# ubuntuslave/vo_single_camera_sos

Hardware: AMD Instinct MI355X
Metric: frame-pairs/sec (detect+match+triangulate+RANSAC) on 640x480 omni, 2000 kpts (higher is better)
Workload: dtype u8/f32/f64

## Files before the change

vo_single_camera_sos_amd/csrc/detect.hip:

```cpp
#include "common.h"

#include <type_traits>

namespace {

constexpr int kThreads = 256;
constexpr int kCandCap = 4096;
constexpr int kCandCapSmall = 2048;
constexpr int kCandCapLarge = 16384;
constexpr int kMaxMasks = 32;

__device__ __forceinline__ float sqrt_rn_normal(float x) {
  const float s = __builtin_amdgcn_sqrtf(x);
  const float s_dn = __int_as_float(__float_as_int(s) - 1), s_up = __int_as_float(__float_as_int(s) + 1);
  const float r_dn = __builtin_fmaf(-s_dn, s, x), r_up = __builtin_fmaf(-s_up, s, x);
  float r = (r_dn <= 0.0f) ? s_dn : s;
  r = (r_up > 0.0f) ? s_up : r;
  return r;
}

constexpr int kEigHalo = 3;
constexpr int kEigStripW = 64 - 2 * kEigHalo;

__device__ __forceinline__ void eig_flush(uint32_t* __restrict__ mstat_img, uint32_t bits, uint32_t omax) {
// ... 71 lines not shown
    if (t > t_last) return;
    const int y_pre = t - 2;
    const bool y_out = y_pre >= ys && y_pre < ye && y_pre >= e_lo && out_lane;
    const uint32_t o_pre = (uint32_t)(max(y_pre, 0) * cols) + (uint32_t)xc;
    const uint32_t mb_pre = y_out ? mb[o_pre] : 0u;
    {
      const int c = c_cur[P];
      const int l = left(c), r = right(c);
      hd[i2] = r - l;
      hs[i2] = (l + 2 * c) + r;
    }
    const int v = t - 1;
    if (v < e_lo - 1) return;
    {
      const int dxi = (hd[i0] + 2 * hd[i1]) + hd[i2], dyi = hs[i2] - hs[i0];
      const float dx = (float)dxi * scale, dy = (float)dyi * scale;
      const float xx = dx * dx, yy = dy * dy;
      float xy = dx * dy;
      if (v < 0 || v >= rows) xy = -xy;
      pxx[i2] = (left(xx) + xx) + right(xx);
      pxy[i2] = (left(xy) + xy) + right(xy);
      pyy[i2] = (left(yy) + yy) + right(yy);
    }
    const int y = v - 1;
    if (y < e_lo) return;
    {
      const float a = ((pxx[i0] + pxx[i1]) + pxx[i2]) * 0.5f, b = (pxy[i0] + pxy[i1]) + pxy[i2];
      const float c = ((pyy[i0] + pyy[i1]) + pyy[i2]) * 0.5f;
      const float e = (a + c) - sqrt_rn_normal(((a - c) * (a - c)) + (b * b));
      if (y_out) {
        const uint32_t bits = mb_pre & mask_all;
        if (bits != cur_bits) {
          eig_flush(mstat_img, cur_bits, cur_max);
          cur_bits = bits;
          cur_max = 0u;
        }
        cur_max = max(cur_max, sosvo_float_ordered(e));
      }
      const float el = left(e), er = right(e);
      hm[i2] = fmaxf(fmaxf(el, e), er);
      ec[i2] = e;
    }
    const int f = y - 1;
    const uint32_t mb_f = mb_prev & mask_all;
    mb_prev = mb_pre;
    if (f < f_lo || f > f_hi) return;
    {
      const float ev = ec[i1];
      const bool is_cand = out_lane && xc >= 1 && xc <= cols - 2 && ev == fmaxf(fmaxf(hm[i0], hm[i1]), hm[i2]) && ev > 0.0f &&
                           mb_f != 0u;
      const unsigned long long bal = __ballot(is_cand);
      if (bal) {
        const int pos = wpos + (int)__builtin_amdgcn_mbcnt_hi((uint32_t)(bal >> 32), __builtin_amdgcn_mbcnt_lo((uint32_t)bal, 0u));
        if (is_cand && pos < wcap) region[pos] = make_uint2(__float_as_uint(ev), (uint32_t)(f * cols + xc));
        wpos += __popcll(bal);
      }
    }
  };
  auto run = [&](auto edge_tag) __attribute__((always_inline)) {
    request(t_first);
    for (int t = t_first; t <= t_last; t += 3) {
#pragma unroll
      for (int k = 0; k < 3; ++k) c_cur[k] = c_pre[k];
      request(t + 3);
      step(std::integral_constant<int, 0>{}, edge_tag, t);
      step(std::integral_constant<int, 1>{}, edge_tag, t + 1);
      step(std::integral_constant<int, 2>{}, edge_tag, t + 2);
    }
  };
  if (edge_strip) run(std::true_type{}); else run(std::false_type{});
  if (lane == 0) wcnt[wave] = (uint32_t)wpos;
  const unsigned long long act = __ballot(out_lane && cur_bits != 0u);
  if (act) {
    const int first = __ffsll((long long)act) - 1;
    const uint32_t b0 = __shfl(cur_bits, first);
    if (__ballot(out_lane && cur_bits != 0u && cur_bits != b0) == 0ULL) {
      uint32_t om = (out_lane && cur_bits != 0u) ? cur_max : 0u;
      for (int s = 32; s > 0; s >>= 1) om = max(om, (uint32_t)__shfl_down((int)om, s));
      if (lane == 0) eig_flush(mstat_img, b0, om);
    } else {
      eig_flush(mstat_img, cur_bits, cur_max);
    }
  }
}

__global__ __launch_bounds__(kThreads) void mask_bbox_kernel(const uint32_t* __restrict__ mask_bits, int images_per_maskset,
                                                             int rows, int cols, int nmask, uint32_t* __restrict__ mstat) {
  __shared__ uint32_t sb[2][kMaxMasks];
  const int tid = threadIdx.x, y = blockIdx.x, set = blockIdx.y;
  if (tid < 2 * kMaxMasks) (&sb[0][0])[tid] = 0u;
  __syncthreads();
  const uint32_t* mb = mask_bits + ((size_t)set * rows + y) * cols;
  const uint32_t mask_all = nmask < 32 ? (1u << nmask) - 1u : 0xFFFFFFFFu;
  for (int x = tid; x < cols; x += kThreads) {
    uint32_t b = mb[x] & mask_all;
    while (b) {
      const int m = __ffs(b) - 1;
      b &= b - 1;
      atomicMax(&sb[0][m], 0xFFFFFFFFu - (uint32_t)x);
      atomicMax(&sb[1][m], (uint32_t)x + 1u);
    }
  }
  __syncthreads();
  if (tid < nmask && sb[1][tid]) {
    uint32_t* st = mstat + ((size_t)set * images_per_maskset * nmask + tid) * 5;
    atomicMax(&st[1], sb[0][tid]);
    atomicMax(&st[2], 0xFFFFFFFFu - (uint32_t)y);
    atomicMax(&st[3], sb[1][tid]);
    atomicMax(&st[4], (uint32_t)y + 1u);
  }
}

template <int LOGR, int NT>
__device__ __forceinline__ void bitonic_pass(unsigned long long* keys, int N, int k, int jtop, int tid) {
  constexpr int R = 1 << LOGR;
  const int jl = jtop >> (LOGR - 1);
  for (int t = tid; t < (N >> LOGR); t += NT) {
    const int i = ((t & ~(jl - 1)) << LOGR) | (t & (jl - 1));
    const bool desc = (i & k) == 0;
    unsigned long long v[R];
#pragma unroll
    for (int m = 0; m < R; ++m) v[m] = keys[i + m * jl];
#pragma unroll
    for (int sb = LOGR - 1; sb >= 0; --sb) {
#pragma unroll
      for (int m = 0; m < R; ++m) {
        if (m & (1 << sb)) continue;
        const unsigned long long a = v[m], b = v[m | (1 << sb)];
        const bool sw = (a < b) == desc;
        v[m] = sw ? b : a;
        v[m | (1 << sb)] = sw ? a : b;
      }
    }
#pragma unroll
    for (int m = 0; m < R; ++m) keys[i + m * jl] = v[m];
  }
}

__device__ __forceinline__ uint32_t dist2_packed(uint32_t a, uint32_t b) {
  typedef short short2v __attribute__((ext_vector_type(2)));
  const short2v d = __builtin_bit_cast(short2v, a) - __builtin_bit_cast(short2v, b);
  return (uint32_t)__builtin_amdgcn_sdot2(d, d, 0, false);
}

struct gft_regions {
  const uint2* cand;
  const uint32_t* wcnt;
  const uint32_t* mb;
  int img, m, strips, nchunks, wcap, s0, c0, ns, R;
  float thr;
};

template <int NT, class F>
__device__ __forceinline__ void gft_walk_keys(const gft_regions& g, int* s_region, int tid, F&& f) {
  const int wave = __builtin_amdgcn_readfirstlane(tid >> 6), lane = tid & 63;
  for (int rb = 0; rb < g.R; rb += NT) {
    if (rb + tid < g.R) {
      const int rg = rb + tid, c = g.c0 + rg / g.ns, sidx = g.s0 + rg % g.ns;
      s_region[tid] = min((int)g.wcnt[(g.img * g.nchunks + c) * g.strips + sidx], g.wcap);
    }
    __syncthreads();
    const int rend = min(NT, g.R - rb);
    for (int rr = wave; rr < rend; rr += NT / 64) {
      const int have = s_region[rr];
      const int rg = rb + rr, c = g.c0 + rg / g.ns, sidx = g.s0 + rg % g.ns;
      const uint2* region = g.cand + (size_t)((g.img * g.nchunks + c) * g.strips + sidx) * g.wcap;
      for (int i = lane; i < have; i += 64) {
        const uint2 r = region[i];
        if (__uint_as_float(r.x) > g.thr && ((g.mb[r.y] >> g.m) & 1u))
          f(((unsigned long long)sosvo_float_ordered(__uint_as_float(r.x)) << 32) | r.y);
      }
    }
    __syncthreads();
  }
}

template <int CAND, int NT>
__device__ __forceinline__ void gft_keep_largest(const gft_regions g, unsigned long long* keys, int* s_region, int* s_count,
                                              int* s_sel, int tid) {
  constexpr int kBits = 11, kBins = 1 << kBits, kPer = kBins / 64;
  static_assert(kBins * sizeof(uint32_t) <= CAND * sizeof(unsigned long long), "the histogram lives in the key LDS");
  uint32_t* hist = reinterpret_cast<uint32_t*>(keys);
  unsigned long long prefix = 0ULL;
  int want = CAND;
  for (int shift = 64; shift > 0;) {
    const int width = min(kBits, shift);
    const unsigned long long high = shift < 64 ? ~0ULL << shift : 0ULL;
    shift -= width;
    for (int i = tid; i < kBins; i += NT) hist[i] = 0u;
    __syncthreads();
    gft_walk_keys<NT>(g, s_region, tid, [&](unsigned long long key) {
      if ((key & high) == prefix) atomicAdd(&hist[(uint32_t)(key >> shift) & ((1u << width) - 1u)], 1u);
    });
    if (tid < 64) {
      uint32_t sum = 0u;
      for (int b = 0; b < kPer; ++b) sum += hist[tid * kPer + b];
      uint32_t incl = sum;
      for (int s = 1; s < 64; s <<= 1) {
        const uint32_t o = (uint32_t)__shfl_down((int)incl, s);
        if (tid + s < 64) incl += o;
      }
      uint32_t above = incl - sum;
      if (above < (uint32_t)want && (uint32_t)want <= incl) {
        for (int b = kPer - 1; b >= 0; --b) {
          const uint32_t c = hist[tid * kPer + b];
          if (above + c >= (uint32_t)want) {
            s_sel[0] = tid * kPer + b;
            s_sel[1] = want - (int)above;
            s_sel[2] = (int)c;
            break;
          }
          above += c;
        }
      }
    }
    __syncthreads();
    prefix |= (unsigned long long)(uint32_t)s_sel[0] << shift;
    want = s_sel[1];
    const bool whole_bin = want == s_sel[2];
    __syncthreads();
    if (whole_bin) break;
  }
// ... 26 lines not shown
  __shared__ unsigned long long lds_u64[CAND];
  __shared__ int s_count, s_accepted, s_overflow;
  __shared__ int s_region[NT];
  __shared__ int s_sel[3];
  __shared__ unsigned long long s_conf[64];
  __shared__ unsigned long long s_prior;
  __shared__ int s_ovf;
  unsigned long long* keys = lds_u64;
  uint32_t* grid = reinterpret_cast<uint32_t*>(lds_u64);
  uint32_t* acc_list = grid + 2 * kSelGridCells;
  const int tid = threadIdx.x;
  const int img = p / nmask, m = p - img * nmask;
  const uint32_t* st = mstat + (size_t)p * 5;
  const uint32_t* sb = mstat + ((size_t)(img / images_per_maskset) * images_per_maskset * nmask + m) * 5;
  uint32_t* sorted = sorted_g + (size_t)p * sorted_stride;
  if (tid == 0) {
    s_count = 0;
    s_accepted = 0;
    s_overflow = 0;
    s_prior = 0ULL;
    s_ovf = 0;
  }
  __syncthreads();
  const bool any = st[0] != 0u;
  const int bx0 = any ? max(1, (int)(0xFFFFFFFFu - sb[1])) : 0, by0 = any ? max(1, (int)(0xFFFFFFFFu - sb[2])) : 0;
  const int bx1 = any ? min(cols - 2, (int)sb[3] - 1) : -1, by1 = any ? min(rows - 2, (int)sb[4] - 1) : -1;
  const int bw = bx1 - bx0 + 1, bh = by1 - by0 + 1;
  if (any && bw > 0 && bh > 0) {
    const float thr = (float)((double)sosvo_ordered_float(st[0]) * quality);
    const uint32_t* mb = mask_bits + (size_t)(img / images_per_maskset) * rows * cols;
    const int s0 = bx0 / kEigStripW, s1 = bx1 / kEigStripW;
    const int c0 = by0 / chunk_rows, c1 = by1 / chunk_rows;
    const int ns = s1 - s0 + 1, R = (c1 - c0 + 1) * ns;
    const int wave = __builtin_amdgcn_readfirstlane(tid >> 6), lane = tid & 63;
    for (int rb = 0; rb < R; rb += NT) {
      if (rb + tid < R) {
        const int rg = rb + tid, c = c0 + rg / ns, sidx = s0 + rg % ns;
        const int have = (int)wcnt[(img * nchunks + c) * strips + sidx];
        if (have > wcap) s_overflow = 1;
        s_region[tid] = min(have, wcap);
      }
      __syncthreads();
      const int rend = min(NT, R - rb);
      for (int rr = wave; rr < rend; rr += NT / 64) {
        const int have = s_region[rr];
        const int rg = rb + rr, c = c0 + rg / ns, sidx = s0 + rg % ns;
        const uint2* region = cand + (size_t)((img * nchunks + c) * strips + sidx) * wcap;
        for (int i0 = 0; i0 < have; i0 += 64) {
          const int i = i0 + lane;
          uint2 r = make_uint2(0u, 0u);
          bool keep = false;
          if (i < have) {
            r = region[i];
            keep = __uint_as_float(r.x) > thr && ((mb[r.y] >> m) & 1u);
          }
          const unsigned long long km = __ballot(keep);
          if (km) {
            const int leader = __ffsll((long long)km) - 1;
            int slot0 = 0;
            if (lane == leader) slot0 = atomicAdd(&s_count, __popcll(km));
            slot0 = __shfl(slot0, leader);
            const int slot = slot0 + __popcll(km & ((1ULL << lane) - 1ULL));
            if (keep && slot < CAND) keys[slot] = ((unsigned long long)sosvo_float_ordered(__uint_as_float(r.x)) << 32) | r.y;
          }
        }
      }
      __syncthreads();
    }
  }
  __syncthreads();
  const int total = s_count;
  if (redo && redo_pass == 0) {
    const int cx0_ = bx0 / cell, cy0_ = by0 / cell;
    const int gw_ = bw > 0 ? bx1 / cell - cx0_ + 1 : 0, gh_ = bh > 0 ? by1 / cell - cy0_ + 1 : 0;
    const bool fits = total <= CAND && (gw_ + 2) * (gh_ + 2) <= kSelGridCells;
    if (tid == 0) redo[p] = fits ? 0 : 1;
    if (!fits) return;
  }
  if (__builtin_expect(total > CAND, 0)) {
    const gft_regions g = {cand, wcnt, mask_bits + (size_t)(img / images_per_maskset) * rows * cols, img, m, strips, nchunks, wcap,
                           bx0 / kEigStripW, by0 / chunk_rows, bx1 / kEigStripW - bx0 / kEigStripW + 1,
                           (by1 / chunk_rows - by0 / chunk_rows + 1) * (bx1 / kEigStripW - bx0 / kEigStripW + 1),
                           (float)((double)sosvo_ordered_float(st[0]) * quality)};
    gft_keep_largest<CAND, NT>(g, keys, s_region, &s_count, s_sel, tid);
    __syncthreads();
  }
  const int n = min(total, CAND);
  int N = 64;
  while (N < n) N <<= 1;
  for (int i = n + tid; i < N; i += NT) keys[i] = 0ULL;
  __syncthreads();
  for (int k = 2, lk = 1; k <= N; k <<= 1, ++lk) {
    for (int left = lk, j = k >> 1; left > 0;) {
      const int take = left >= 3 ? 3 : left;
      if (take == 3) bitonic_pass<3, NT>(keys, N, k, j, tid);
      else if (take == 2) bitonic_pass<2, NT>(keys, N, k, j, tid);
      else bitonic_pass<1, NT>(keys, N, k, j, tid);
      j >>= take;
      left -= take;
      __syncthreads();
    }
  }
  for (int i = tid; i < n; i += NT) {
    const uint32_t pix = (uint32_t)keys[i];
    const uint32_t y = pix / (uint32_t)cols;
    sorted[i] = (y << 16) | (pix - y * (uint32_t)cols);
  }
  int stt = (total > CAND || s_overflow) ? 1 : 0;
  const int cx0 = bx0 / cell, cy0 = by0 / cell;
  const int gw = bw > 0 ? bx1 / cell - cx0 + 1 : 0, gh = bh > 0 ? by1 / cell - cy0 + 1 : 0;
  const bool use_grid = gw * gh <= kSelGridCells;
  const int limit_list = 1024;
  const float md2 = min_distance * min_distance;
  const bool spaced = min_distance >= 1.0f;
  int limit = cap;
  if (max_corners > 0 && max_corners < limit) limit = max_corners;
  constexpr uint32_t kEmpty = 0xFFFFFFFFu;
  const int gwp = gw + 2;
  const bool fast = NT > 256 && spaced && n > 0 && cell <= 2048 && rows <= 32768 && cols <= 32768 && gwp * (gh + 2) <= kSelGridCells;
  __syncthreads();
  if (fast) {
    for (int i = tid; i < gwp * (gh + 2) * 2; i += NT) grid[i] = kEmpty;
  } else {
    for (int i = tid; i < (use_grid ? gw * gh * 2 : 0); i += NT) grid[i] = 0u;
  }
  __syncthreads();
  if (fast) {
    const int wave = __builtin_amdgcn_readfirstlane(tid >> 6), lane = tid & 63;
    const uint32_t thr_i = (uint32_t)ceilf(md2);
    const uint32_t magic = cell > 1 ? 0xFFFFFFFFu / (uint32_t)cell + 1u : 0u;
    int accepted = 0;
    uint32_t xy_next = lane < n ? sorted[lane] : 0u;
    for (int k0 = 0; k0 < n && accepted < limit; k0 += 64) {
      const int kend = min(64, n - k0);
      const bool active = lane < kend;
      const uint32_t xy = xy_next;
      xy_next = k0 + 64 + lane < n ? sorted[k0 + 64 + lane] : 0u;
      const int y = (int)(xy >> 16), x = (int)(xy & 0xFFFFu);
      const int xc = active ? (int)(cell > 1 ? __umulhi((uint32_t)x, magic) : (uint32_t)x) - cx0 + 1 : 1;
      const int yc = active ? (int)(cell > 1 ? __umulhi((uint32_t)y, magic) : (uint32_t)y) - cy0 + 1 : 1;
      const int cidx = (yc * gwp + xc) * 2;
      constexpr int NWV = NT / 64;
      for (int c9 = wave; c9 < 9; c9 += NWV) {
        const uint2 q2 = *reinterpret_cast<const uint2*>(&grid[cidx + (c9 / 3 - 1) * gwp * 2 + (c9 % 3 - 1) * 2]);
        const uint32_t hit = ((uint32_t)(q2.x != kEmpty) & (uint32_t)(dist2_packed(xy, q2.x) < thr_i)) |
                             ((uint32_t)(q2.y != kEmpty) & (uint32_t)(dist2_packed(xy, q2.y) < thr_i));
        const unsigned long long hb = __ballot(active && hit != 0u);
        if (hb && lane == 0) atomicOr(&s_prior, hb);
      }
      for (int a = wave, novf = min(s_ovf, limit_list); a < novf; a += NWV) {
        const unsigned long long hb = __ballot(active && dist2_packed(xy, acc_list[a]) < thr_i);
        if (hb && lane == 0) atomicOr(&s_prior, hb);
      }
      {
        const int first = (wave + NWV - 9 % NWV) % NWV;
        uint32_t glo = 0u, ghi = 0u;
        int t = 0;
        for (int jb = first; jb < kend; jb += 4 * NWV, t += 4) {
#pragma unroll
          for (int u = 0; u < 4; ++u) {
            const int j = min(jb + u * NWV, 63);
            const unsigned long long row = __ballot(active && dist2_packed(xy, (uint32_t)__builtin_amdgcn_readlane((int)xy, j)) < thr_i);
            const bool here = lane == t + u;
            glo = here ? (uint32_t)row : glo;
            ghi = here ? (uint32_t)(row >> 32) : ghi;
          }
        }
        const int jmine = first + lane * NWV;
        if (jmine < kend) s_conf[jmine] = ((unsigned long long)ghi << 32) | glo;
      }
      __syncthreads();
      if (wave == 0) {
        const unsigned long long alive0 = __ballot(active) & ~s_prior;
        const unsigned long long mine = active ? s_conf[lane] : 0ULL;
        const unsigned long long lt = (1ULL << lane) - 1ULL;
        const bool surv = (alive0 >> lane) & 1ULL;
        const unsigned long long fr = __ballot(surv && (mine & alive0 & lt) == 0ULL);
        unsigned long long pending = alive0 & ~fr, acc = fr;
        const int rlo = (int)(uint32_t)mine, rhi = (int)(uint32_t)(mine >> 32);
        while (pending) {
          const int j = __ffsll((long long)pending) - 1;
          pending &= pending - 1ULL;
          const unsigned long long row = ((unsigned long long)(uint32_t)__builtin_amdgcn_readlane(rhi, j) << 32) |
                                         (uint32_t)__builtin_amdgcn_readlane(rlo, j);
          if ((row & acc & ((1ULL << j) - 1ULL)) == 0ULL) acc |= 1ULL << j;
        }
        const int room = limit - accepted;
        acc = __ballot(((acc >> lane) & 1ULL) && __popcll(acc & lt) < room);
        if ((acc >> lane) & 1ULL) {
          const int pos = accepted + __popcll(acc & ((1ULL << lane) - 1ULL));
          kp[((size_t)p * cap + pos) * 2] = (float)x;
          kp[((size_t)p * cap + pos) * 2 + 1] = (float)y;
          if (atomicCAS(&grid[cidx], kEmpty, xy) != kEmpty && atomicCAS(&grid[cidx + 1], kEmpty, xy) != kEmpty) {
            const int o = atomicAdd(&s_ovf, 1);
            if (o < limit_list) acc_list[o] = xy;
          }
        }
        if (lane == 0) {
          s_accepted = accepted + __popcll(acc);
          s_prior = 0ULL;
        }
      }
      __syncthreads();
      accepted = s_accepted;
    }
    if (s_ovf > limit_list) stt |= 2;
  } else
  if (tid < 64) {
    const int lane = tid;
    if (!use_grid && limit_list < limit) {
      limit = limit_list;
      stt |= 2;
    }
    int accepted = 0;
    uint32_t xy_next = lane < n ? sorted[lane] : 0u;
    for (int k0 = 0; k0 < n && accepted < limit; k0 += 64) {
      const int kend = min(64, n - k0);
      const bool active = lane < kend;
      const uint32_t xy = xy_next;
      xy_next = k0 + 64 + lane < n ? sorted[k0 + 64 + lane] : 0u;
      const int y = (int)(xy >> 16), x = (int)(xy & 0xFFFFu);
      bool prior = false;
      if (active && spaced) {
        if (use_grid) {
          const int xc = x / cell - cx0, yc = y / cell - cy0;
#pragma unroll
          for (int c9 = 0; c9 < 9; ++c9) {
            const int xx = xc + (c9 % 3) - 1, yy = yc + (c9 / 3) - 1;
            if (xx < 0 || xx >= gw || yy < 0 || yy >= gh) continue;
            const uint2 q2 = *reinterpret_cast<const uint2*>(&grid[(yy * gw + xx) * 2]);
#pragma unroll
            for (int slot = 0; slot < 2; ++slot) {
              const uint32_t q = slot ? q2.y : q2.x;
              if (q) {
                const float dx = (float)(x - (int)((q - 1u) & 0xFFFFu)), dy = (float)(y - (int)((q - 1u) >> 16));
                prior = prior || (dx * dx + dy * dy < md2);
              }
            }
          }
          for (int a = 0, novf = min(s_ovf, limit_list); a < novf; ++a) {
            const uint32_t q = acc_list[a];
            const float dx = (float)(x - (int)(q & 0xFFFFu)), dy = (float)(y - (int)(q >> 16));
            prior = prior || (dx * dx + dy * dy < md2);
          }
        } else {
          for (int a = 0; a < accepted; ++a) {
            const uint32_t q = acc_list[a];
            const float dx = (float)(x - (int)(q & 0xFFFFu)), dy = (float)(y - (int)(q >> 16));
            prior = prior || (dx * dx + dy * dy < md2);
          }
        }
      }
      unsigned long long alive = __ballot(active && !prior);
      unsigned long long acc = 0ULL;
      int room = limit - accepted;
      while (alive && room > 0) {
        const int j = __ffsll((long long)alive) - 1;
        alive &= alive - 1ULL;
        acc |= 1ULL << j;
// ... 58 lines not shown
    if (ys >= ye) return;
  }
  const uint8_t* g = gray + (size_t)img * img_stride;
  uint8_t* o = out + (size_t)img * out_stride;
  uint32_t h[7] = {0, 0, 0, 0, 0, 0, 0};
  const bool edge_strip = xb < 3 || xb + 64 > cols - 3;
  const int t_first = ys - 3, t_last = ye + 2;
  int c_pre[7];
  auto request = [&](int t0, int k0, int k1) __attribute__((always_inline)) {
#pragma unroll
    for (int k = 0; k < 7; ++k)
      if (k >= k0 && k < k1) c_pre[k] = (int)g[(uint32_t)(refl101(min(t0 + k, t_last), rows) * cols) + (uint32_t)xs];
  };
  request(t_first, 0, 7);
  auto step = [&](auto phase_tag, auto edge_tag, const int t) __attribute__((always_inline)) {
    constexpr int P = decltype(phase_tag)::value;
    constexpr bool EDGE = decltype(edge_tag)::value;
    if (t > t_last) return;
    const int c = c_pre[P];
    int l1, l2, l3, r1, r2, r3;
    if (EDGE) {
      l3 = __shfl(c, src[0]); l2 = __shfl(c, src[1]); l1 = __shfl(c, src[2]);
      r1 = __shfl(c, src[4]); r2 = __shfl(c, src[5]); r3 = __shfl(c, src[6]);
    } else {
      l1 = lane_from_left(c); l2 = lane_from_left(l1); l3 = lane_from_left(l2);
      r1 = lane_from_right(c); r2 = lane_from_right(r1); r3 = lane_from_right(r2);
    }
    h[P] = vmad24(18u, (uint32_t)(l3 + r3), vmad24(34u, (uint32_t)(l2 + r2), vmad24(49u, (uint32_t)(l1 + r1), 54u * (uint32_t)c)));
    const int y = t - 3;
    if (y < ys) return;
    const uint32_t vsum = vmad24(18u, h[(P + 1) % 7] + h[P], vmad24(34u, h[(P + 2) % 7] + h[(P + 6) % 7],
                                vmad24(49u, h[(P + 3) % 7] + h[(P + 5) % 7], 54u * h[(P + 4) % 7])));
    if (out_lane) o[(uint32_t)(y * cols) + (uint32_t)xc] = (uint8_t)((vsum + 32768u) >> 16);
  };
  auto run = [&](auto edge_tag) __attribute__((always_inline)) {
    for (int t = t_first; t <= t_last; t += 7) {
      step(std::integral_constant<int, 0>{}, edge_tag, t);
      step(std::integral_constant<int, 1>{}, edge_tag, t + 1);
      step(std::integral_constant<int, 2>{}, edge_tag, t + 2);
      step(std::integral_constant<int, 3>{}, edge_tag, t + 3);
      request(t + 7, 0, 4);
      step(std::integral_constant<int, 4>{}, edge_tag, t + 4);
      step(std::integral_constant<int, 5>{}, edge_tag, t + 5);
      step(std::integral_constant<int, 6>{}, edge_tag, t + 6);
      request(t + 7, 4, 7);
    }
  };
  if (edge_strip) run(std::true_type{}); else run(std::false_type{});
}

constexpr int kPatchMaxR = 23, kPatchRows = 48, kPatchStride = 64;
constexpr int kDescRegionBytesGft = 24 * 1024;
typedef uint32_t __attribute__((aligned(1))) u32_unaligned;
template <int NT>
__global__ __launch_bounds__(NT) void orb_describe_kernel(const uint8_t* __restrict__ blurred, int rows, int cols,
                                                                int nmask, int cap, float* __restrict__ kp,
                                                                int32_t* __restrict__ n_io, float cos_a, float sin_a,
                                                                const int8_t* __restrict__ pattern, int edge,
                                                                uint8_t* __restrict__ desc, int nimg_total,
                                                                const int32_t* __restrict__ row_range, int imgs_per_range) {
  SOSVO_LATENCY_BOUND_PRIO();
  extern __shared__ float lds_kp[];
  __shared__ int off[512];
  __shared__ uint16_t poff[512];
  constexpr int kPatchWords = (NT / 64) * (kPatchRows * kPatchStride / 4);
  constexpr int kRegionWords = NT == 256 ? kDescRegionBytesGft / 4 : 0;
  __shared__ uint32_t patch_area[kPatchWords > kRegionWords ? kPatchWords : kRegionWords];
  __shared__ int wave_off[NT / 64 + 1];
  __shared__ int s_running, s_R;
  __shared__ int s_bb[4];
  const int tid = threadIdx.x, lane = tid & 63, wid = tid >> 6;
  const int p = xcd_problem(nimg_total, nmask);
  if (p < 0) return;
  const int img = p / nmask;
  const int n = min(n_io[p], cap);
  if (tid == 0) {
    s_running = 0;
    s_R = 0;
  }
  __syncthreads();
  for (int i = tid; i < 512; i += NT) {
    const float px = (float)pattern[2 * i], py = (float)pattern[2 * i + 1];
    const float xr = (px * cos_a) - (py * sin_a), yr = (px * sin_a) + (py * cos_a);
    const int dx = __float2int_rn(xr), dy = __float2int_rn(yr);
    off[i] = dy * cols + dx;
    atomicMax(&s_R, max(abs(dx), abs(dy)));
  }
  __syncthreads();
  const int R = s_R;
  const bool patch_ok = R <= kPatchMaxR && edge >= R + 1;
  const int PR = 2 * R + 1;
  int y_first = 0, y_last = rows - 1;
  if (row_range) {
    const int v = img / imgs_per_range;
    const int rr_lo = row_range[2 * v], rr_hi = row_range[2 * v + 1];
    y_first = (rr_lo <= 0 ? 0 : rr_lo + 3) + R;
    y_last = (rr_hi >= rows ? rows : rr_hi - 3) - 1 - R;
  }
  const int pdw = (PR + 3) >> 2;
  const int pstride = pdw | 1;
  if (patch_ok)
    for (int i = tid; i < 512; i += NT) {
      const int dy = (off[i] + R * cols + R) / cols - R;
      const int dx = off[i] - dy * cols;
      poff[i] = (uint16_t)((dy + R) * (4 * pstride) + (dx + R));
    }
  for (int i0 = 0; i0 < n; i0 += NT) {
    const int i = i0 + tid;
    float x = 0.f, y = 0.f;
    bool keep = false;
    if (i < n) {
      x = kp[((size_t)p * cap + i) * 2];
      y = kp[((size_t)p * cap + i) * 2 + 1];
      keep = x >= (float)edge && x < (float)(cols - edge) && y >= (float)edge && y < (float)(rows - edge);
      const int yi = __float2int_rn(y);
      keep = keep && yi >= y_first && yi <= y_last;
    }
    const int pos = sosvo_block_compact_pos<NT / 64>(keep, wave_off, &s_running, tid);
    if (keep) {
      lds_kp[2 * pos] = x;
      lds_kp[2 * pos + 1] = y;
    }
  }
  __syncthreads();
  const int m = s_running;
  for (int i = tid; i < 2 * m; i += NT) kp[(size_t)p * cap * 2 + i] = lds_kp[i];
  if (tid == 0) n_io[p] = m;
  const uint8_t* im = blurred + (size_t)img * rows * cols;
  if constexpr (NT == 256) {
    if (patch_ok && m > 0) {
      if (tid < 4) s_bb[tid] = tid < 2 ? 0x7FFFFFFF : -1;
      __syncthreads();
      for (int i = tid; i < m; i += NT) {
        const int cx = __float2int_rn(lds_kp[2 * i]), cy = __float2int_rn(lds_kp[2 * i + 1]);
        atomicMin(&s_bb[0], cx);
        atomicMin(&s_bb[1], cy);
        atomicMax(&s_bb[2], cx);
        atomicMax(&s_bb[3], cy);
      }
      __syncthreads();
      const int rx0 = s_bb[0] - R, ry0 = s_bb[1] - R, rw = s_bb[2] - s_bb[0] + PR, rh = s_bb[3] - s_bb[1] + PR;
      const int ldw = (rw + 3) >> 2, pitch_dw = ldw | 1, pitch_b = 4 * pitch_dw;
      if (pitch_b * rh <= kDescRegionBytesGft) {
        {
          const int step_r = NT / ldw, step_k = NT - step_r * ldw;
          int ry = tid / ldw, k = tid - ry * ldw;
          const uint8_t* org = im + (size_t)ry0 * cols + rx0;
          while (__any(ry < rh)) {
            uint32_t v[8];
            int dst[8];
#pragma unroll
            for (int u = 0; u < 8; ++u) {
              dst[u] = ry < rh ? ry * pitch_dw + k : -1;
              v[u] = *reinterpret_cast<const u32_unaligned*>(org + (uint32_t)(min(ry, rh - 1) * cols + 4 * k));
              k += step_k;
              ry += step_r;
              if (k >= ldw) {
                k -= ldw;
                ++ry;
              }
            }
#pragma unroll
            for (int u = 0; u < 8; ++u)
              if (dst[u] >= 0) patch_area[dst[u]] = v[u];
          }
        }
        int ra[4], rb[4];
#pragma unroll
        for (int r = 0; r < 4; ++r) {
#pragma unroll
          for (int e = 0; e < 2; ++e) {
            const int o = off[2 * (64 * r + lane) + e];
            const int dy = (o + R * cols + R) / cols - R, dx = o - dy * cols;
            (e ? rb[r] : ra[r]) = dy * pitch_b + dx;
          }
        }
        __syncthreads();
        const uint8_t* region8 = reinterpret_cast<const uint8_t*>(patch_area);
        const int wid_s = __builtin_amdgcn_readfirstlane(wid);
        for (int j = wid_s; j < m; j += NT / 64) {
          const int cx = __builtin_amdgcn_readfirstlane(__float2int_rn(lds_kp[2 * j]));
          const int cy = __builtin_amdgcn_readfirstlane(__float2int_rn(lds_kp[2 * j + 1]));
          const int org = (cy - ry0) * pitch_b + (cx - rx0);
          unsigned long long* d = reinterpret_cast<unsigned long long*>(desc + ((size_t)p * cap + j) * 32);
          unsigned long long mine = 0ULL;
#pragma unroll
          for (int r = 0; r < 4; ++r) {
            const unsigned long long bal = __ballot(region8[org + ra[r]] < region8[org + rb[r]]);
            if (lane == r) mine = bal;
          }
          if (lane < 4) d[lane] = mine;
        }
        return;
      }
      __syncthreads();
    }
  }
  if (patch_ok) {
    uint32_t* patch32 = patch_area + wid * (kPatchRows * kPatchStride / 4);
    const uint8_t* patch = reinterpret_cast<const uint8_t*>(patch32);
    const int lsh = pdw <= 8 ? 3 : 4;
    const int prow = lane >> lsh, pk = min(lane & ((1 << lsh) - 1), pdw - 1);
    const int rpr = 64 >> lsh, nit = (PR + rpr - 1) / rpr;
    uint32_t reg[kPatchRows / 4];
    int goff[kPatchRows / 4], lidx[kPatchRows / 4];
#pragma unroll
    for (int it = 0; it < kPatchRows / 4; ++it) {
      const int r = min(rpr * it + prow, PR - 1);
      goff[it] = r * cols;
      lidx[it] = r * pstride + pk;
    }
    auto issue = [&](int j) {
      const uint8_t* base =
          im + ((size_t)__float2int_rn(lds_kp[2 * j + 1]) - R) * cols + (__float2int_rn(lds_kp[2 * j]) - R) + 4 * pk;
#pragma unroll
      for (int it = 0; it < kPatchRows / 4; ++it)
        if (it < nit) reg[it] = *reinterpret_cast<const u32_unaligned*>(base + goff[it]);
    };
    int pa[4], pb[4];
#pragma unroll
    for (int r = 0; r < 4; ++r) {
      pa[r] = poff[2 * (64 * r + lane)];
      pb[r] = poff[2 * (64 * r + lane) + 1];
    }
    int j = wid;
    if (j < m) issue(j);
    for (; j < m; j += NT / 64) {
#pragma unroll
      for (int it = 0; it < kPatchRows / 4; ++it)
        if (it < nit) patch32[lidx[it]] = reg[it];
      if (j + NT / 64 < m) issue(j + NT / 64);
      unsigned long long* d = reinterpret_cast<unsigned long long*>(desc + ((size_t)p * cap + j) * 32);
      unsigned long long mine = 0ULL;
#pragma unroll
      for (int r = 0; r < 4; ++r) {
        const unsigned long long bal = __ballot(patch[pa[r]] < patch[pb[r]]);
        if (lane == r) mine = bal;
      }
      if (lane < 4) d[lane] = mine;
    }
    return;
  }
  for (int j = wid; j < m; j += NT / 64) {
    const uint8_t* c = im + (size_t)__float2int_rn(lds_kp[2 * j + 1]) * cols + __float2int_rn(lds_kp[2 * j]);
    unsigned long long* d = reinterpret_cast<unsigned long long*>(desc + ((size_t)p * cap + j) * 32);
#pragma unroll
    for (int r = 0; r < 4; ++r) {
      const int t = 64 * r + lane;
      const unsigned long long bal = __ballot(c[off[2 * t]] < c[off[2 * t + 1]]);
      if (lane == 0) d[r] = bal;
    }
  }
}

static void rolling_chunks(int nimg, int rows, int strips, int* nchunks, int* chunk_rows) {
  int nc = cdiv(16384, nimg * strips);
  if (nc > rows / 24) nc = rows / 24;
  if (nc < 1) nc = 1;
  *chunk_rows = cdiv(rows, nc);
  *nchunks = cdiv(rows, *chunk_rows);
}

}

static int32_t launch_gauss7_rows(sosvo_ctx* ctx, const uint8_t* in, long long in_stride, int nimg, int rows, int cols,
                                  uint8_t* out, long long out_stride, const int32_t* row_range, int imgs_per_range) {
  const int strips = cdiv(cols, kEigStripW);
  int nchunks, chunk_rows;
  rolling_chunks(nimg, rows, strips, &nchunks, &chunk_rows);
  SOSVO_LAUNCH(ctx, gauss7_kernel, dim3(cdiv(nimg * strips * nchunks, kThreads / 64)), dim3(kThreads), 0, ctx->stream, in,
               in_stride, nimg, rows, cols, strips, nchunks, chunk_rows, out, out_stride, row_range, imgs_per_range);
  SOSVO_LAUNCH_CHECK(ctx);
  return SOSVO_OK;
}
int32_t sosvo_launch_gauss7_rows(sosvo_ctx* ctx, const uint8_t* in, long long in_stride, int nimg, int rows, int cols,
                                 uint8_t* out, long long out_stride, const int32_t* row_range, int imgs_per_range) {
  return launch_gauss7_rows(ctx, in, in_stride, nimg, rows, cols, out, out_stride, row_range, imgs_per_range);
}
int32_t sosvo_launch_gauss7_to(sosvo_ctx* ctx, const uint8_t* in, long long in_stride, int nimg, int rows, int cols,
                               uint8_t* out, long long out_stride) {
  return launch_gauss7_rows(ctx, in, in_stride, nimg, rows, cols, out, out_stride, nullptr, 1);
}
int32_t sosvo_launch_gauss7(sosvo_ctx* ctx, const uint8_t* in, long long img_stride, int nimg, int rows, int cols,
                            uint8_t* out) {
  return sosvo_launch_gauss7_to(ctx, in, img_stride, nimg, rows, cols, out, img_stride);
}

extern "C" {

int32_t sosvo_detect_gft(sosvo_ctx* ctx, const uint8_t* gray, const uint32_t* mask_bits, int32_t nimg,
                         int32_t images_per_maskset, int32_t rows, int32_t cols, int32_t nmask, double quality,
                         double min_distance, int32_t max_corners, int32_t cap, float* kp, int32_t* n,
                         int32_t* status) {
  SOSVO_ENTER(ctx);
  SOSVO_REQUIRE(ctx, gray && mask_bits && kp && n, "null pointer");
  SOSVO_REQUIRE(ctx, nimg >= 0 && nimg <= 65535 && images_per_maskset > 0, "nimg out of range");
  SOSVO_REQUIRE(ctx, rows >= 3 && cols >= 3 && rows * (int64_t)cols < (1 << 28), "image sizes out of range");
  SOSVO_REQUIRE(ctx, nmask >= 1 && nmask <= kMaxMasks, "nmask out of range (1..32)");
  SOSVO_REQUIRE(ctx, cap > 0 && cap <= 4096 && quality > 0 && min_distance >= 0, "bad detector parameters (quality > 0)");
  if (nimg == 0) return SOSVO_OK;
  const size_t P = (size_t)nimg * nmask;
  size_t off = 0;
  auto carve = [&](size_t bytes) {
    size_t o = off;
    off += (bytes + 255) & ~(size_t)255;
    return o;
  };
  const int strips = cdiv(cols, kEigStripW);
  int nchunks, chunk_rows;
  rolling_chunks(nimg, rows, strips, &nchunks, &chunk_rows);
  const int wcap = (chunk_rows * kEigStripW + 63) & ~63;
  const size_t n_waves = (size_t)nimg * strips * nchunks;
  const size_t o_cand = carve(sizeof(uint2) * n_waves * wcap);
  const size_t o_wcnt = carve(sizeof(uint32_t) * n_waves);
  const size_t o_stat = carve(sizeof(uint32_t) * P * 5);
  const bool large = cap > 1024;
  const int sorted_stride = large ? kCandCapLarge : kCandCap;
  const size_t o_sorted = carve(sizeof(uint32_t) * P * sorted_stride);
  const size_t o_redo = carve(sizeof(int32_t) * P);
  int32_t rc = sosvo_ws_reserve(ctx, off);
  if (rc != SOSVO_OK) return rc;
  char* ws = (char*)ctx->ws;
  uint2* cand = (uint2*)(ws + o_cand);
  uint32_t* wcnt = (uint32_t*)(ws + o_wcnt);
  uint32_t* mstat = (uint32_t*)(ws + o_stat);
  uint32_t* sorted_g = (uint32_t*)(ws + o_sorted);
  SOSVO_HIP(ctx, hipMemsetAsync(mstat, 0, sizeof(uint32_t) * P * 5, ctx->stream));

  const int nsets = cdiv(nimg, images_per_maskset);
  SOSVO_LAUNCH(ctx, mask_bbox_kernel, dim3(rows, nsets), dim3(kThreads), 0, ctx->stream, mask_bits, images_per_maskset, rows,
               cols, nmask, mstat);
  SOSVO_LAUNCH_CHECK(ctx);
  const int waves = nimg * strips * nchunks;
  SOSVO_LAUNCH(ctx, min_eigen_kernel, dim3(cdiv(waves, kThreads / 64)), dim3(kThreads), 0, ctx->stream, gray, mask_bits, nimg,
               images_per_maskset, rows, cols, nmask, strips, nchunks, chunk_rows, wcap, cand, wcnt, mstat);
  SOSVO_LAUNCH_CHECK(ctx);
  const int cell = min_distance >= 1 ? (int)lrint(min_distance) : 1;
  int32_t* redo = (int32_t*)(ws + o_redo);
  if (large) {
    SOSVO_PROFILE(ctx, "gft_select_kernel");
    hipLaunchKernelGGL((gft_select_kernel<kCandCapLarge, 1024>), dim3(xcd_grid(nimg, nmask)), dim3(1024), 0, ctx->stream, cand, wcnt,
                       strips, nchunks, chunk_rows, wcap, mask_bits, mstat, images_per_maskset, nmask, rows, cols, quality, (float)min_distance, cell,
                       max_corners, cap, sorted_g, sorted_stride, kp, n, status, nullptr, 0, nimg);
  } else {
    SOSVO_PROFILE(ctx, "gft_select_kernel");
    auto launch = [&](auto small, auto full, int nt) {
      hipLaunchKernelGGL(small, dim3(xcd_grid(nimg, nmask)), dim3(nt), 0, ctx->stream, cand, wcnt, strips, nchunks, chunk_rows, wcap,
                         mask_bits, mstat, images_per_maskset, nmask, rows, cols, quality, (float)min_distance, cell, max_corners, cap,
                         sorted_g, sorted_stride, kp, n, status, redo, 0, nimg);
      hipLaunchKernelGGL(full, dim3(xcd_grid(nimg, nmask)), dim3(nt), 0, ctx->stream, cand, wcnt, strips, nchunks, chunk_rows, wcap,
                         mask_bits, mstat, images_per_maskset, nmask, rows, cols, quality, (float)min_distance, cell, max_corners, cap,
                         sorted_g, sorted_stride, kp, n, status, redo, 1, nimg);
    };
    if (P <= 1024)
      launch(gft_select_kernel<kCandCapSmall, 512>, gft_select_kernel<kCandCap, 512>, 512);
    else
      launch(gft_select_kernel<kCandCapSmall, kThreads>, gft_select_kernel<kCandCap, kThreads>, kThreads);
  }
  SOSVO_LAUNCH_CHECK(ctx);
  return SOSVO_OK;
}

int32_t sosvo_describe_orb(sosvo_ctx* ctx, const uint8_t* gray, int32_t nimg, int32_t rows, int32_t cols,
                           int32_t nmask, int32_t cap, float* kp, int32_t* n, float cos_a, float sin_a,
                           const int8_t* pattern, int32_t edge, uint8_t* desc) {
  return sosvo_describe_orb_rows(ctx, gray, nimg, rows, cols, nmask, cap, kp, n, cos_a, sin_a, pattern, edge, nullptr, desc);
}

int32_t sosvo_describe_orb_rows(sosvo_ctx* ctx, const uint8_t* gray, int32_t nimg, int32_t rows, int32_t cols,
                                int32_t nmask, int32_t cap, float* kp, int32_t* n, float cos_a, float sin_a,
                                const int8_t* pattern, int32_t edge, const int32_t* row_range, uint8_t* desc) {
  SOSVO_ENTER(ctx);
  SOSVO_REQUIRE(ctx, row_range == nullptr || nimg % 2 == 0, "row_range needs the two views' images (nimg even, view-major)");
  SOSVO_REQUIRE(ctx, gray && kp && n && pattern && desc, "null pointer");
  SOSVO_REQUIRE(ctx, nimg >= 0 && nimg <= 65535 && nmask >= 1, "nimg / nmask out of range");
  SOSVO_REQUIRE(ctx, rows >= 1 && cols >= 1 && rows * (int64_t)cols < (1 << 28), "image sizes out of range");
  SOSVO_REQUIRE(ctx, cap > 0 && cap <= 4096, "cap out of range");
  SOSVO_REQUIRE(ctx, edge >= 19, "edge must cover the rotated 31x31 patch (>= 19)");
  SOSVO_REQUIRE(ctx, ((uintptr_t)desc & 7) == 0, "desc must be 8-byte aligned");
  if (nimg == 0) return SOSVO_OK;
  const size_t bytes = (size_t)nimg * rows * cols;
  int32_t rc = sosvo_ws_reserve(ctx, bytes);
  if (rc != SOSVO_OK) return rc;
  uint8_t* blurred = (uint8_t*)ctx->ws;
  rc = launch_gauss7_rows(ctx, gray, (long long)rows * cols, nimg, rows, cols, blurred, (long long)rows * cols, row_range,
                          nimg > 1 ? nimg / 2 : 1);
  if (rc != SOSVO_OK) return rc;
  const size_t lds_kp_bytes = (size_t)cap * 2 * sizeof(float);
  const int irange = nimg > 1 ? nimg / 2 : 1;
  SOSVO_PROFILE(ctx, "orb_describe_kernel");
  auto launch = [&](auto kernel, int nt) {
    hipLaunchKernelGGL(kernel, dim3(xcd_grid(nimg, nmask)), dim3(nt), lds_kp_bytes, ctx->stream, blurred, rows, cols, nmask, cap, kp,
                       n, cos_a, sin_a, pattern, edge, desc, nimg, row_range, irange);
  };
  if (cap > 1024)
    launch(orb_describe_kernel<1024>, 1024);
  else if ((size_t)nimg * nmask <= 1024)
    launch(orb_describe_kernel<512>, 512);
  else
    launch(orb_describe_kernel<kThreads>, kThreads);
  SOSVO_LAUNCH_CHECK(ctx);
  return SOSVO_OK;
}

}
```

Baseline: 64410.

## Pack candidates as y<<16|x, add grid-based NMS for small blocks, precompute ORB pattern table

```diff
diff --git a/vo_single_camera_sos_amd/csrc/detect.hip b/vo_single_camera_sos_amd/csrc/detect.hip
--- a/vo_single_camera_sos_amd/csrc/detect.hip
+++ b/vo_single_camera_sos_amd/csrc/detect.hip
@@ -147,7 +147,7 @@
       const unsigned long long bal = __ballot(is_cand);
       if (bal) {
         const int pos = wpos + (int)__builtin_amdgcn_mbcnt_hi((uint32_t)(bal >> 32), __builtin_amdgcn_mbcnt_lo((uint32_t)bal, 0u));
-        if (is_cand && pos < wcap) region[pos] = make_uint2(__float_as_uint(ev), (uint32_t)(f * cols + xc));
+        if (is_cand && pos < wcap) region[pos] = make_uint2(__float_as_uint(ev), ((uint32_t)f << 16) | (uint32_t)xc);
         wpos += __popcll(bal);
       }
     }
@@ -238,11 +238,40 @@
   return (uint32_t)__builtin_amdgcn_sdot2(d, d, 0, false);
 }
 
+constexpr uint32_t kGridEmpty = 0xFFFFFFFFu;
+struct gft_igrid {
+  uint32_t thr_i;
+  uint32_t magic;
+  int cell, cx0, cy0, gwp;
+  __device__ __forceinline__ gft_igrid(float md2, int cell_, int cx0_, int cy0_, int gwp_)
+      : thr_i((uint32_t)__builtin_amdgcn_readfirstlane((int)(uint32_t)ceilf(md2))),
+        magic((uint32_t)__builtin_amdgcn_readfirstlane((int)(cell_ > 1 ? 0xFFFFFFFFu / (uint32_t)cell_ + 1u : 0u))), cell(cell_),
+        cx0(cx0_), cy0(cy0_), gwp(gwp_) {}
+  __device__ __forceinline__ int cell_index(uint32_t xy, bool active) const {
+    const uint32_t x = xy & 0xFFFFu, y = xy >> 16;
+    const int xc = active ? (int)(cell > 1 ? __umulhi(x, magic) : x) - cx0 + 1 : 1;
+    const int yc = active ? (int)(cell > 1 ? __umulhi(y, magic) : y) - cy0 + 1 : 1;
+    return (yc * gwp + xc) * 2;
+  }
+  __device__ __forceinline__ uint32_t cell_hit(const uint32_t* grid, int cidx, int dxc, int dyc, uint32_t xy) const {
+    const uint2 q2 = *reinterpret_cast<const uint2*>(&grid[cidx + dyc * gwp * 2 + dxc * 2]);
+    return ((uint32_t)(q2.x != kGridEmpty) & (uint32_t)(dist2_packed(xy, q2.x) < thr_i)) |
+           ((uint32_t)(q2.y != kGridEmpty) & (uint32_t)(dist2_packed(xy, q2.y) < thr_i));
+  }
+  __device__ __forceinline__ bool near(uint32_t a, uint32_t b) const { return dist2_packed(a, b) < thr_i; }
+  __device__ __forceinline__ void insert(uint32_t* grid, int cidx, uint32_t xy, int* s_ovf, uint32_t* acc_list, int limit_list) const {
+    if (atomicCAS(&grid[cidx], kGridEmpty, xy) != kGridEmpty && atomicCAS(&grid[cidx + 1], kGridEmpty, xy) != kGridEmpty) {
+      const int o = atomicAdd(s_ovf, 1);
+      if (o < limit_list) acc_list[o] = xy;
+    }
+  }
+};
+
 struct gft_regions {
   const uint2* cand;
   const uint32_t* wcnt;
   const uint32_t* mb;
-  int img, m, strips, nchunks, wcap, s0, c0, ns, R;
+  int img, m, cols, strips, nchunks, wcap, s0, c0, ns, R;
   float thr;
 };
 
@@ -262,7 +291,7 @@
       const uint2* region = g.cand + (size_t)((g.img * g.nchunks + c) * g.strips + sidx) * g.wcap;
       for (int i = lane; i < have; i += 64) {
         const uint2 r = region[i];
-        if (__uint_as_float(r.x) > g.thr && ((g.mb[r.y] >> g.m) & 1u))
+        if (__uint_as_float(r.x) > g.thr && ((g.mb[(r.y >> 16) * (uint32_t)g.cols + (r.y & 0xFFFFu)] >> g.m) & 1u))
           f(((unsigned long long)sosvo_float_ordered(__uint_as_float(r.x)) << 32) | r.y);
       }
     }
@@ -395,7 +424,7 @@
           bool keep = false;
           if (i < have) {
             r = region[i];
-            keep = __uint_as_float(r.x) > thr && ((mb[r.y] >> m) & 1u);
+            keep = __uint_as_float(r.x) > thr && ((mb[(r.y >> 16) * (uint32_t)cols + (r.y & 0xFFFFu)] >> m) & 1u);
           }
           const unsigned long long km = __ballot(keep);
           if (km) {
@@ -421,7 +450,7 @@
     if (!fits) return;
   }
   if (__builtin_expect(total > CAND, 0)) {
-    const gft_regions g = {cand, wcnt, mask_bits + (size_t)(img / images_per_maskset) * rows * cols, img, m, strips, nchunks, wcap,
+    const gft_regions g = {cand, wcnt, mask_bits + (size_t)(img / images_per_maskset) * rows * cols, img, m, cols, strips, nchunks, wcap,
                            bx0 / kEigStripW, by0 / chunk_rows, bx1 / kEigStripW - bx0 / kEigStripW + 1,
                            (by1 / chunk_rows - by0 / chunk_rows + 1) * (bx1 / kEigStripW - bx0 / kEigStripW + 1),
                            (float)((double)sosvo_ordered_float(st[0]) * quality)};
@@ -444,11 +473,7 @@
       __syncthreads();
     }
   }
-  for (int i = tid; i < n; i += NT) {
-    const uint32_t pix = (uint32_t)keys[i];
-    const uint32_t y = pix / (uint32_t)cols;
-    sorted[i] = (y << 16) | (pix - y * (uint32_t)cols);
-  }
+  for (int i = tid; i < n; i += NT) sorted[i] = (uint32_t)keys[i];
   int stt = (total > CAND || s_overflow) ? 1 : 0;
   const int cx0 = bx0 / cell, cy0 = by0 / cell;
   const int gw = bw > 0 ? bx1 / cell - cx0 + 1 : 0, gh = bh > 0 ? by1 / cell - cy0 + 1 : 0;
@@ -458,20 +483,19 @@
   const bool spaced = min_distance >= 1.0f;
   int limit = cap;
   if (max_corners > 0 && max_corners < limit) limit = max_corners;
-  constexpr uint32_t kEmpty = 0xFFFFFFFFu;
   const int gwp = gw + 2;
-  const bool fast = NT > 256 && spaced && n > 0 && cell <= 2048 && rows <= 32768 && cols <= 32768 && gwp * (gh + 2) <= kSelGridCells;
-  __syncthreads();
-  if (fast) {
-    for (int i = tid; i < gwp * (gh + 2) * 2; i += NT) grid[i] = kEmpty;
+  const bool igrid = spaced && n > 0 && cell <= 2048 && rows <= 32768 && cols <= 32768 && gwp * (gh + 2) <= kSelGridCells;
+  const bool fast = NT > 256 && igrid;
+  __syncthreads();
+  if (igrid) {
+    for (int i = tid; i < gwp * (gh + 2) * 2; i += NT) grid[i] = kGridEmpty;
   } else {
     for (int i = tid; i < (use_grid ? gw * gh * 2 : 0); i += NT) grid[i] = 0u;
   }
   __syncthreads();
   if (fast) {
     const int wave = __builtin_amdgcn_readfirstlane(tid >> 6), lane = tid & 63;
-    const uint32_t thr_i = (uint32_t)ceilf(md2);
-    const uint32_t magic = cell > 1 ? 0xFFFFFFFFu / (uint32_t)cell + 1u : 0u;
+    const gft_igrid ig(md2, cell, cx0, cy0, gwp);
     int accepted = 0;
     uint32_t xy_next = lane < n ? sorted[lane] : 0u;
     for (int k0 = 0; k0 < n && accepted < limit; k0 += 64) {
@@ -480,19 +504,14 @@
       const uint32_t xy = xy_next;
       xy_next = k0 + 64 + lane < n ? sorted[k0 + 64 + lane] : 0u;
       const int y = (int)(xy >> 16), x = (int)(xy & 0xFFFFu);
-      const int xc = active ? (int)(cell > 1 ? __umulhi((uint32_t)x, magic) : (uint32_t)x) - cx0 + 1 : 1;
-      const int yc = active ? (int)(cell > 1 ? __umulhi((uint32_t)y, magic) : (uint32_t)y) - cy0 + 1 : 1;
-      const int cidx = (yc * gwp + xc) * 2;
+      const int cidx = ig.cell_index(xy, active);
       constexpr int NWV = NT / 64;
       for (int c9 = wave; c9 < 9; c9 += NWV) {
-        const uint2 q2 = *reinterpret_cast<const uint2*>(&grid[cidx + (c9 / 3 - 1) * gwp * 2 + (c9 % 3 - 1) * 2]);
-        const uint32_t hit = ((uint32_t)(q2.x != kEmpty) & (uint32_t)(dist2_packed(xy, q2.x) < thr_i)) |
-                             ((uint32_t)(q2.y != kEmpty) & (uint32_t)(dist2_packed(xy, q2.y) < thr_i));
-        const unsigned long long hb = __ballot(active && hit != 0u);
+        const unsigned long long hb = __ballot(active && ig.cell_hit(grid, cidx, c9 % 3 - 1, c9 / 3 - 1, xy) != 0u);
         if (hb && lane == 0) atomicOr(&s_prior, hb);
       }
       for (int a = wave, novf = min(s_ovf, limit_list); a < novf; a += NWV) {
-        const unsigned long long hb = __ballot(active && dist2_packed(xy, acc_list[a]) < thr_i);
+        const unsigned long long hb = __ballot(active && ig.near(xy, acc_list[a]));
         if (hb && lane == 0) atomicOr(&s_prior, hb);
       }
       {
@@ -503,7 +522,7 @@
 #pragma unroll
           for (int u = 0; u < 4; ++u) {
             const int j = min(jb + u * NWV, 63);
-            const unsigned long long row = __ballot(active && dist2_packed(xy, (uint32_t)__builtin_amdgcn_readlane((int)xy, j)) < thr_i);
+            const unsigned long long row = __ballot(active && ig.near(xy, (uint32_t)__builtin_amdgcn_readlane((int)xy, j)));
             const bool here = lane == t + u;
             glo = here ? (uint32_t)row : glo;
             ghi = here ? (uint32_t)(row >> 32) : ghi;
@@ -534,10 +553,7 @@
           const int pos = accepted + __popcll(acc & ((1ULL << lane) - 1ULL));
           kp[((size_t)p * cap + pos) * 2] = (float)x;
           kp[((size_t)p * cap + pos) * 2 + 1] = (float)y;
-          if (atomicCAS(&grid[cidx], kEmpty, xy) != kEmpty && atomicCAS(&grid[cidx + 1], kEmpty, xy) != kEmpty) {
-            const int o = atomicAdd(&s_ovf, 1);
-            if (o < limit_list) acc_list[o] = xy;
-          }
+          ig.insert(grid, cidx, xy, &s_ovf, acc_list, limit_list);
         }
         if (lane == 0) {
           s_accepted = accepted + __popcll(acc);
@@ -548,6 +564,44 @@
       accepted = s_accepted;
     }
     if (s_ovf > limit_list) stt |= 2;
+  } else if (NT <= 256 && igrid) {
+    if (tid < 64) {
+      const int lane = tid;
+      const gft_igrid ig(md2, cell, cx0, cy0, gwp);
+      int accepted = 0;
+      uint32_t xy_next = lane < n ? sorted[lane] : 0u;
+      for (int k0 = 0; k0 < n && accepted < limit; k0 += 64) {
+        const int kend = min(64, n - k0);
+        const bool active = lane < kend;
+        const uint32_t xy = xy_next;
+        xy_next = k0 + 64 + lane < n ? sorted[k0 + 64 + lane] : 0u;
+        const int cidx = ig.cell_index(xy, active);
+        uint32_t prior = 0u;
+#pragma unroll 1
+        for (int dyc = -1; dyc <= 1; ++dyc)
+#pragma unroll
+          for (int dxc = -1; dxc <= 1; ++dxc) prior |= ig.cell_hit(grid, cidx, dxc, dyc, xy);
+        for (int a = 0, novf = min(s_ovf, limit_list); a < novf; ++a) prior |= (uint32_t)ig.near(xy, acc_list[a]);
+        unsigned long long alive = __ballot(active && prior == 0u);
+        unsigned long long acc = 0ULL;
+        int room = limit - accepted;
+        while (alive && room > 0) {
+          const int j = __ffsll((long long)alive) - 1;
+          alive &= alive - 1ULL;
+          acc |= 1ULL << j;
+          room--;
+          alive &= ~__ballot(ig.near(xy, (uint32_t)__builtin_amdgcn_readlane((int)xy, j)));
+        }
+        if ((acc >> lane) & 1ULL) {
+          const int pos = accepted + __popcll(acc & ((1ULL << lane) - 1ULL));
+          kp[((size_t)p * cap + pos) * 2] = (float)(xy & 0xFFFFu);
+          kp[((size_t)p * cap + pos) * 2 + 1] = (float)(xy >> 16);
+          ig.insert(grid, cidx, xy, &s_ovf, acc_list, limit_list);
+        }
+        accepted += __popcll(acc);
+      }
+      if (lane == 0) s_accepted = accepted;
+    }
   } else
   if (tid < 64) {
     const int lane = tid;
@@ -712,42 +766,69 @@
 constexpr int kPatchMaxR = 23, kPatchRows = 48, kPatchStride = 64;
 constexpr int kDescRegionBytesGft = 24 * 1024;
 typedef uint32_t __attribute__((aligned(1))) u32_unaligned;
+
+__host__ __device__ __forceinline__ int orb_patch_stride_dw(int R) { return ((2 * R + 1 + 3) >> 2) | 1; }
+struct orb_pattern_table {
+  int2 pt[256];
+  int R, pad;
+  uint16_t poff[512];
+};
+__global__ __launch_bounds__(256) void orb_pattern_table_kernel(const int8_t* __restrict__ pattern, float cos_a, float sin_a,
+                                                                orb_pattern_table* __restrict__ tab) {
+  __shared__ int s_R;
+  const int t = threadIdx.x;
+  if (t == 0) s_R = 0;
+  __syncthreads();
+  int d[4];
+#pragma unroll
+  for (int e = 0; e < 2; ++e) {
+    const float px = (float)pattern[4 * t + 2 * e], py = (float)pattern[4 * t + 2 * e + 1];
+    const float xr = (px * cos_a) - (py * sin_a), yr = (px * sin_a) + (py * cos_a);
+    d[2 * e] = __float2int_rn(xr);
+    d[2 * e + 1] = __float2int_rn(yr);
+  }
+  tab->pt[t] = make_int2((int)(((uint32_t)d[1] << 16) | ((uint32_t)d[0] & 0xFFFFu)), (int)(((uint32_t)d[3] << 16) | ((uint32_t)d[2] & 0xFFFFu)));
+  atomicMax(&s_R, max(max(abs(d[0]), abs(d[1])), max(abs(d[2]), abs(d[3]))));
+  __syncthreads();
+  const int R = s_R;
+  if (t == 0) tab->R = R;
+  const int pitch = R <= kPatchMaxR ? 4 * orb_patch_stride_dw(R) : 0;
+  tab->poff[2 * t] = (uint16_t)(R <= kPatchMaxR ? (d[1] + R) * pitch + (d[0] + R) : 0);
+  tab->poff[2 * t + 1] = (uint16_t)(R <= kPatchMaxR ? (d[3] + R) * pitch + (d[2] + R) : 0);
+}
+
 template <int NT>
 __global__ __launch_bounds__(NT) void orb_describe_kernel(const uint8_t* __restrict__ blurred, int rows, int cols,
                                                                 int nmask, int cap, float* __restrict__ kp,
-                                                                int32_t* __restrict__ n_io, float cos_a, float sin_a,
-                                                                const int8_t* __restrict__ pattern, int edge,
+                                                                int32_t* __restrict__ n_io, const orb_pattern_table* __restrict__ ptab, int edge,
                                                                 uint8_t* __restrict__ desc, int nimg_total,
                                                                 const int32_t* __restrict__ row_range, int imgs_per_range) {
   SOSVO_LATENCY_BOUND_PRIO();
   extern __shared__ float lds_kp[];
-  __shared__ int off[512];
-  __shared__ uint16_t poff[512];
   constexpr int kPatchWords = (NT / 64) * (kPatchRows * kPatchStride / 4);
   constexpr int kRegionWords = NT == 256 ? kDescRegionBytesGft / 4 : 0;
   __shared__ uint32_t patch_area[kPatchWords > kRegionWords ? kPatchWords : kRegionWords];
   __shared__ int wave_off[NT / 64 + 1];
-  __shared__ int s_running, s_R;
+  __shared__ int s_running;
   __shared__ int s_bb[4];
   const int tid = threadIdx.x, lane = tid & 63, wid = tid >> 6;
   const int p = xcd_problem(nimg_total, nmask);
   if (p < 0) return;
   const int img = p / nmask;
   const int n = min(n_io[p], cap);
-  if (tid == 0) {
-    s_running = 0;
-    s_R = 0;
-  }
-  __syncthreads();
-  for (int i = tid; i < 512; i += NT) {
-    const float px = (float)pattern[2 * i], py = (float)pattern[2 * i + 1];
-    const float xr = (px * cos_a) - (py * sin_a), yr = (px * sin_a) + (py * cos_a);
-    const int dx = __float2int_rn(xr), dy = __float2int_rn(yr);
-    off[i] = dy * cols + dx;
-    atomicMax(&s_R, max(abs(dx), abs(dy)));
-  }
-  __syncthreads();
-  const int R = s_R;
+  if (tid == 0) s_running = 0;
+  __syncthreads();
+  const int R = ptab->R;
+  auto lane_offsets = [&](int pitch, int* a, int* b) __attribute__((always_inline)) {
+    const int2* tp = ptab->pt;
+    asm volatile("" : "+s"(tp));
+#pragma unroll
+    for (int r = 0; r < 4; ++r) {
+      const int2 d = tp[64 * r + lane];
+      a[r] = (d.x >> 16) * pitch + (int)(short)d.x;
+      b[r] = (d.y >> 16) * pitch + (int)(short)d.y;
+    }
+  };
   const bool patch_ok = R <= kPatchMaxR && edge >= R + 1;
   const int PR = 2 * R + 1;
   int y_first = 0, y_last = rows - 1;
@@ -758,13 +839,7 @@
     y_last = (rr_hi >= rows ? rows : rr_hi - 3) - 1 - R;
   }
   const int pdw = (PR + 3) >> 2;
-  const int pstride = pdw | 1;
-  if (patch_ok)
-    for (int i = tid; i < 512; i += NT) {
-      const int dy = (off[i] + R * cols + R) / cols - R;
-      const int dx = off[i] - dy * cols;
-      poff[i] = (uint16_t)((dy + R) * (4 * pstride) + (dx + R));
-    }
+  const int pstride = orb_patch_stride_dw(R);
   for (int i0 = 0; i0 < n; i0 += NT) {
     const int i = i0 + tid;
     float x = 0.f, y = 0.f;
@@ -826,15 +901,7 @@
           }
         }
         int ra[4], rb[4];
-#pragma unroll
-        for (int r = 0; r < 4; ++r) {
-#pragma unroll
-          for (int e = 0; e < 2; ++e) {
-            const int o = off[2 * (64 * r + lane) + e];
-            const int dy = (o + R * cols + R) / cols - R, dx = o - dy * cols;
-            (e ? rb[r] : ra[r]) = dy * pitch_b + dx;
-          }
-        }
+        lane_offsets(pitch_b, ra, rb);
         __syncthreads();
         const uint8_t* region8 = reinterpret_cast<const uint8_t*>(patch_area);
         const int wid_s = __builtin_amdgcn_readfirstlane(wid);
@@ -880,8 +947,8 @@
     int pa[4], pb[4];
 #pragma unroll
     for (int r = 0; r < 4; ++r) {
-      pa[r] = poff[2 * (64 * r + lane)];
-      pb[r] = poff[2 * (64 * r + lane) + 1];
+      pa[r] = ptab->poff[2 * (64 * r + lane)];
+      pb[r] = ptab->poff[2 * (64 * r + lane) + 1];
     }
     int j = wid;
     if (j < m) issue(j);
@@ -901,13 +968,14 @@
     }
     return;
   }
+  int ga[4], gb[4];
+  lane_offsets(cols, ga, gb);
   for (int j = wid; j < m; j += NT / 64) {
     const uint8_t* c = im + (size_t)__float2int_rn(lds_kp[2 * j + 1]) * cols + __float2int_rn(lds_kp[2 * j]);
     unsigned long long* d = reinterpret_cast<unsigned long long*>(desc + ((size_t)p * cap + j) * 32);
 #pragma unroll
     for (int r = 0; r < 4; ++r) {
-      const int t = 64 * r + lane;
-      const unsigned long long bal = __ballot(c[off[2 * t]] < c[off[2 * t + 1]]);
+      const unsigned long long bal = __ballot(c[ga[r]] < c[gb[r]]);
       if (lane == 0) d[r] = bal;
     }
   }
@@ -956,6 +1024,7 @@
   SOSVO_REQUIRE(ctx, gray && mask_bits && kp && n, "null pointer");
   SOSVO_REQUIRE(ctx, nimg >= 0 && nimg <= 65535 && images_per_maskset > 0, "nimg out of range");
   SOSVO_REQUIRE(ctx, rows >= 3 && cols >= 3 && rows * (int64_t)cols < (1 << 28), "image sizes out of range");
+  SOSVO_REQUIRE(ctx, rows <= 65535 && cols <= 65535, "image sizes out of range (the candidates are packed as y << 16 | x)");
   SOSVO_REQUIRE(ctx, nmask >= 1 && nmask <= kMaxMasks, "nmask out of range (1..32)");
   SOSVO_REQUIRE(ctx, cap > 0 && cap <= 4096 && quality > 0 && min_distance >= 0, "bad detector parameters (quality > 0)");
   if (nimg == 0) return SOSVO_OK;
@@ -1040,9 +1109,13 @@
   SOSVO_REQUIRE(ctx, ((uintptr_t)desc & 7) == 0, "desc must be 8-byte aligned");
   if (nimg == 0) return SOSVO_OK;
   const size_t bytes = (size_t)nimg * rows * cols;
-  int32_t rc = sosvo_ws_reserve(ctx, bytes);
+  const size_t o_tab = (bytes + 255) & ~(size_t)255;
+  int32_t rc = sosvo_ws_reserve(ctx, o_tab + sizeof(orb_pattern_table));
   if (rc != SOSVO_OK) return rc;
   uint8_t* blurred = (uint8_t*)ctx->ws;
+  orb_pattern_table* ptab = (orb_pattern_table*)((char*)ctx->ws + o_tab);
+  SOSVO_LAUNCH(ctx, orb_pattern_table_kernel, dim3(1), dim3(256), 0, ctx->stream, pattern, cos_a, sin_a, ptab);
+  SOSVO_LAUNCH_CHECK(ctx);
   rc = launch_gauss7_rows(ctx, gray, (long long)rows * cols, nimg, rows, cols, blurred, (long long)rows * cols, row_range,
                           nimg > 1 ? nimg / 2 : 1);
   if (rc != SOSVO_OK) return rc;
@@ -1051,7 +1124,7 @@
   SOSVO_PROFILE(ctx, "orb_describe_kernel");
   auto launch = [&](auto kernel, int nt) {
     hipLaunchKernelGGL(kernel, dim3(xcd_grid(nimg, nmask)), dim3(nt), lds_kp_bytes, ctx->stream, blurred, rows, cols, nmask, cap, kp,
-                       n, cos_a, sin_a, pattern, edge, desc, nimg, row_range, irange);
+                       n, ptab, edge, desc, nimg, row_range, irange);
   };
   if (cap > 1024)
     launch(orb_describe_kernel<1024>, 1024);
```

After: 66640, median of 6. 1.03x the previous value.
